# F-Fer/SLAM-Loop-Closing

Hardware: AMD Instinct MI355X
Metric: Hamming distances/sec (256-bit ORB) for all-vs-all loop search, 1/2/4/8 GPUs (higher is better)
Workload: dtype u32

## Files before the change

include/lcm.h:

```cpp
#ifndef LCM_H_
#define LCM_H_

#include <stddef.h>
#include <stdint.h>

#ifdef __cplusplus
extern "C" {
#endif

#if defined(__GNUC__)
#define LCM_API __attribute__((visibility("default")))
#else
#define LCM_API
#endif

#define LCM_DESC_BYTES 32
#define LCM_DESC_WORDS 8
#define LCM_MAX_TRAIN_ROWS (1 << 22)

typedef enum lcm_status {
    LCM_OK = 0,
    LCM_ERR_INVALID_ARG = -1,
    LCM_ERR_NO_DEVICE = -2,
    LCM_ERR_HIP = -3,
// ... 275 lines not shown
LCM_API int  lcm_group_sync(lcm_group* g);
LCM_API int  lcm_group_set_tuning(lcm_group* g, int knob, int value);
LCM_API int  lcm_group_set_kernel_variant(lcm_group* g, int variant);
LCM_API int  lcm_group_all_vs_all(lcm_group* g, lcm_score* out_scores, size_t cap, size_t* n_pairs, size_t* pair_offsets);
LCM_API int  lcm_group_all_vs_all_argmin(lcm_group* g, lcm_score* out_scores, uint32_t* out_index_sums, size_t cap,
                                         size_t* n_pairs, size_t* pair_offsets);
LCM_API int  lcm_group_all_vs_all_loops(lcm_group* g, lcm_loop_candidate* out, size_t cap, size_t* n_out, size_t* n_pairs_out);
LCM_API int  lcm_group_all_vs_all_ratio(lcm_group* g, double ratio, lcm_score* out_scores, size_t cap, size_t* n_pairs,
                                        size_t* pair_offsets);
LCM_API int  lcm_group_all_vs_all_loops_ratio(lcm_group* g, const lcm_ratio_loop_params* rp, lcm_loop_candidate* out,
                                              size_t cap, size_t* n_out, size_t* n_pairs_out);
LCM_API int  lcm_group_last_info(const lcm_group* g, lcm_group_info* info);
LCM_API int  lcm_group_query_scores(lcm_group* g, const uint8_t* query, int nq, int query_frame_id,
                                    lcm_score* out_scores, int32_t* out_frame_ids, int cap, int* n_out);
LCM_API int  lcm_group_query_scores_batch(lcm_group* g, const uint8_t* const* queries, const int* nq,
                                          const int* query_frame_ids, int n_queries,
                                          lcm_score* out_scores, size_t cap, size_t* n_out, size_t* offsets);
LCM_API int  lcm_group_query_submit_batch(lcm_group* g, const uint8_t* const* queries, const int* nq,
                                          const int* query_frame_ids, int n_queries, int* ticket);
LCM_API int  lcm_group_query_collect_batch(lcm_group* g, int ticket, lcm_score* out_scores, size_t cap, size_t* n_out,
                                           size_t* offsets);
LCM_API int  lcm_group_online_stats_read(lcm_group* g, lcm_online_stats* out, int reset);
LCM_API int  lcm_group_detect_loops(lcm_group* g, int current_frame_id, const uint8_t* query, int nq, int n_keypoints,
                                    lcm_loop_candidate* out, int cap, int* n_out);
LCM_API int  lcm_merge_shard_scores(const lcm_score* const* shard_scores, const size_t* shard_counts, int world,
                                    const int32_t* ids, int n_frames, int min_gap,
                                    lcm_score* out, size_t cap, size_t* n_out, size_t* offsets);

LCM_API int  lcm_merge_shard_scores_device(lcm_handle* h, const void* d_gathered, const size_t* shard_counts, int world,
                                           const int32_t* ids, int n_frames, int min_gap,
                                           void* d_merged, size_t cap, size_t* n_out);

typedef enum lcm_tuning { LCM_TUNE_ITEM_SLOTS = 0, LCM_TUNE_ONLINE_SPLIT = 1, LCM_TUNE_PACKED = 2, LCM_TUNE_ONLINE_STREAMS = 3,
                          LCM_TUNE_PACKED_SCRATCH_MB = 4, LCM_TUNE_PAIR_UPLOAD_KERNEL = 5, LCM_TUNE_PAIR_HOST_FOLD = 6 } lcm_tuning;
LCM_API int  lcm_set_tuning(lcm_handle* h, int knob, int value);

LCM_API int  lcm_dev_alloc(lcm_handle* h, size_t bytes, void** d_ptr);
LCM_API int  lcm_dev_free(lcm_handle* h, void* d_ptr);
LCM_API int  lcm_dev_upload(lcm_handle* h, void* d_dst, const void* src, size_t bytes);
LCM_API int  lcm_dev_download(lcm_handle* h, void* dst, const void* d_src, size_t bytes);

#ifdef __cplusplus
}
#endif
#endif
```

slam-loop-closing_amd/capi.py:

```python
from __future__ import annotations

import ctypes as C
import os
from typing import Optional, Sequence, Tuple

import numpy as np

_HERE = os.path.dirname(os.path.abspath(__file__))
LIB_PATH = os.environ.get("LCM_LIB_PATH") or os.path.join(_HERE, "lib", "liblcm_hip.so")
DESC_BYTES = 32
SIFT_BYTES = 128
KEY_SHIFT = 22
TUNE_ITEM_SLOTS, TUNE_ONLINE_SPLIT, TUNE_PACKED, TUNE_ONLINE_STREAMS, TUNE_PACKED_SCRATCH_MB = 0, 1, 2, 3, 4
TUNE_PAIR_UPLOAD_KERNEL, TUNE_PAIR_HOST_FOLD = 5, 6


OK, ERR_INVALID_ARG, ERR_NO_DEVICE, ERR_HIP, ERR_CAPACITY, ERR_ORDER, ERR_NOT_FOUND, ERR_OOM = 0, -1, -2, -3, -4, -5, -6, -7


class LcmError(RuntimeError):
    def __init__(self, code: int, msg: str):
        super().__init__(f"lcm error {code}: {msg}")
        self.code = code


class Params(C.Structure):
    _fields_ = [("ratio", C.c_int32), ("dist_floor", C.c_int32), ("min_matches", C.c_int32),
                ("min_gap", C.c_int32), ("sim_threshold", C.c_double), ("cross_check", C.c_int32),
                ("reserved", C.c_int32)]


class Score(C.Structure):
    _fields_ = [("good_count", C.c_uint32), ("min_dist", C.c_uint16), ("n_train", C.c_uint16)]


class DMatch(C.Structure):
    _fields_ = [("query_idx", C.c_int32), ("train_idx", C.c_int32), ("img_idx", C.c_int32), ("distance", C.c_float)]


class LoopCandidate(C.Structure):
    _fields_ = [("current_frame_id", C.c_int32), ("matched_frame_id", C.c_int32), ("num_matches", C.c_int32),
                ("similarity_score", C.c_double)]


class RatioLoopParams(C.Structure):
    _fields_ = [("ratio", C.c_double), ("min_rows", C.c_int32), ("min_matches", C.c_int32)]

# ... 1346 lines not shown
```

slam-loop-closing_amd/csrc/lcm_api.cpp:

```cpp
#include "lcm_internal.h"

namespace lcm {
std::string& last_error() { static thread_local std::string e; return e; }
int fail(int code, const char* fmt, ...) {
    char buf[512];
    va_list ap;
    va_start(ap, fmt);
    vsnprintf(buf, sizeof buf, fmt, ap);
    va_end(ap);
    last_error() = buf;
    return code;
}
void set_last_error(const char* msg) { last_error() = msg ? msg : ""; }
}

namespace lcm {

int set_device(const lcm_handle* h) {
    HIP_TRY(hipSetDevice(h->device));
    return LCM_OK;
}

int wait_db(lcm_handle* h) {
    if (h->pending_copy) {
// ... 247 lines not shown

int lcm_set_kernel_variant(lcm_handle* h, int variant) {
    if (!h) return fail(LCM_ERR_INVALID_ARG, "NULL handle");
    if (variant < 0 || variant > 5) return fail(LCM_ERR_INVALID_ARG, "unknown kernel variant %d", variant);
    h->variant = variant;
    return LCM_OK;
}

int lcm_set_tuning(lcm_handle* h, int knob, int value) {
    if (!h) return fail(LCM_ERR_INVALID_ARG, "NULL handle");
    switch (knob) {
        case LCM_TUNE_ITEM_SLOTS:
            if (value < 0 || value > 64) return fail(LCM_ERR_INVALID_ARG, "item slots must be 0 (automatic) .. 64");
            h->tune_item_slots = value; h->plan.key = 0; return LCM_OK;
        case LCM_TUNE_ONLINE_SPLIT:
            if (value != -1 && value != 0 && value != 1 && value != 2 && value != 4 && value != 16 && value != 32)
                return fail(LCM_ERR_INVALID_ARG, "online split must be -1 (automatic), 0 (off), 1, 2, 4 (rows per lane of a 256-thread workgroup), 16 or 32 (64 / 128 threads x 8 rows)");
            h->tune_online_split = value; return LCM_OK;
        case LCM_TUNE_ONLINE_STREAMS:
            if (value != 0 && value != 1) return fail(LCM_ERR_INVALID_ARG, "online streams must be 0 (the handle's stream) or 1 (one per query slot)");
            h->tune_online_streams = value; return LCM_OK;
        case LCM_TUNE_PAIR_UPLOAD_KERNEL:
            if (value != 0 && value != 1) return fail(LCM_ERR_INVALID_ARG, "pair upload must be 0 (hipMemcpyAsync) or 1 (kernel)");
            h->tune_pair_upload_kernel = value; return LCM_OK;
        case LCM_TUNE_PAIR_HOST_FOLD:
            if (value != 0 && value != 1) return fail(LCM_ERR_INVALID_ARG, "pair host fold must be 0 (device buffer + copy) or 1 (pinned host memory)");
            h->tune_pair_host_fold = value; return LCM_OK;
        case LCM_TUNE_PACKED_SCRATCH_MB:
            if (value < 1 || value > 65536) return fail(LCM_ERR_INVALID_ARG, "packed scratch must be 1 .. 65536 MiB per chunk");
            h->pk_scratch_cfg_words = h->pk_scratch_words = (size_t)value << 18; h->plan.key = 0; return LCM_OK;
        case LCM_TUNE_PACKED:
            if (value < -1 || value > 2) return fail(LCM_ERR_INVALID_ARG, "packed rows must be -1 (automatic), 0 (off), 1 (on) or 2 (on, 1536-row columns)");
            h->tune_packed = value; h->plan.key = 0; return LCM_OK;
        default: return fail(LCM_ERR_INVALID_ARG, "unknown tuning knob %d", knob);
    }
}


static int db_reserve_impl(lcm_handle* h, int n_frames, int max_desc) {
    if (!h || n_frames < 0 || max_desc < 0) return fail(LCM_ERR_INVALID_ARG, "bad argument");
    if (max_desc > MAX_FRAME_ROWS) return fail(LCM_ERR_CAPACITY, "a stored frame may hold at most %d rows (got %d)", MAX_FRAME_ROWS, max_desc);
    int rc = set_device(h); if (rc) return rc;
    return grow_arena(h, std::max(n_frames, 1), std::max(max_desc, 1));
}

static int db_append_impl(lcm_handle* h, int frame_id, const uint8_t* desc, int n, int n_keypoints) {
    if (!h || (n > 0 && !desc)) return fail(LCM_ERR_INVALID_ARG, "NULL argument");
    int rc = set_device(h); if (rc) return rc;
    rc = check_append(h, frame_id, n); if (rc) return rc;
    const int slot = (int)h->frames.size();
    const int b = h->stage_next;
    h->stage_next = (b + 1) % STAGE_BUFS;
    HIP_TRY(hipEventSynchronize(h->stage_done[b]));
    const int np = padded_rows(n);
    if (n > 0) {
        memcpy(h->h_stage[b], desc, (size_t)n * LCM_DESC_BYTES);
        for (int r = n; r < np; ++r) memcpy(h->h_stage[b] + (size_t)r * LCM_DESC_BYTES, desc + (size_t)(n - 1) * LCM_DESC_BYTES, LCM_DESC_BYTES);
        HIP_TRY(hipMemcpyAsync(h->d_rows + (size_t)slot * h->stride_rows * LCM_DESC_BYTES, h->h_stage[b],
                               (size_t)np * LCM_DESC_BYTES, hipMemcpyHostToDevice, h->copy_stream));
    }
    h->h_counts[slot] = n;
    HIP_TRY(hipMemcpyAsync(h->d_counts + slot, h->h_counts + slot, sizeof(int32_t), hipMemcpyHostToDevice, h->copy_stream));
    HIP_TRY(hipEventRecord(h->stage_done[b], h->copy_stream));
    HIP_TRY(hipEventRecord(h->db_ready, h->copy_stream));
    h->pending_copy = true; h->db_ready_recorded = true;
    h->frames.push_back({frame_id, n, n_keypoints < 0 ? n : n_keypoints});
// ... 259 lines not shown
```

slam-loop-closing_amd/csrc/lcm_bulk.cpp:

```cpp
#include "lcm_internal.h"

namespace {

struct PackedPlan {
    std::vector<uint32_t> tab;
    std::vector<lcm::WorkItem> items;
    std::vector<Plan::PackedChunk> chunks;
    size_t max_pairs = 0;
    uint64_t lane_slots = 0;
};

constexpr int PK_GROUP_FRAMES = 256;

int build_packed_plan(const std::vector<size_t>& offsets, const std::vector<int32_t>& qn, const uint32_t* q_frame_of, int chunk,
                      uint32_t COL, uint32_t stride, size_t scratch_words, PackedPlan& pk) {
    const size_t budget = std::max<size_t>(1, scratch_words / stride);
    const int n_q = (int)qn.size();
    auto elig_of = [&](int c) { return (uint32_t)(offsets[(size_t)c + 1] - offsets[(size_t)c]); };
    pk.tab.resize((size_t)n_q * 2 + 1);
    for (int c = 0; c <= n_q; ++c) pk.tab[(size_t)c] = (uint32_t)offsets[(size_t)c];
    for (int c = 0; c < n_q; ++c) pk.tab[(size_t)n_q + 1 + (size_t)c] = (uint32_t)qn[(size_t)c];
    std::vector<int> pos;
    struct Col { uint32_t w, k, me; };
    std::vector<Col> cols;
    bool first_chunk = offsets[(size_t)n_q] > budget;
    int c0 = 0;
    while (c0 < n_q) {
        const int min_frames = (int)std::max<size_t>(1, std::min<size_t>((size_t)PK_GROUP_FRAMES, budget / (size_t)std::max(chunk, 1)));
        int c1 = c0;
        size_t pairs = 0;
        while (c1 < n_q && (c1 - c0 < min_frames || pairs + elig_of(c1) <= budget)) { pairs += elig_of(c1); ++c1; }
        pos.clear();
        for (int c = c0; c < c1; ++c) if (elig_of(c) > 0) pos.push_back(c);
        c0 = c1;
        if (pos.empty()) continue;
        std::stable_sort(pos.begin(), pos.end(), [&](int x, int y) { return elig_of(x) > elig_of(y); });
        const size_t np = pos.size();
        const uint32_t tab0 = (uint32_t)pk.tab.size();
        pk.tab.resize(pk.tab.size() + 4 * np + 1);
        uint32_t* vstart = pk.tab.data() + tab0;
        uint32_t* qframe = vstart + np + 1;
        uint32_t* eligp = qframe + np;
        uint32_t* cidx = eligp + np;
        uint64_t v = 0;
// ... 26 lines not shown
            ch.item0 = (uint32_t)pk.items.size(); ch.tab0 = tab0; ch.ptab0 = (uint32_t)pk.tab.size(); ch.n_pos = (uint32_t)np; ch.slot0 = s0;
            pk.tab.resize(pk.tab.size() + np + 1);
            {
                uint32_t* pairsp = pk.tab.data() + ch.ptab0;
                size_t t = 0;
                for (size_t q = 0; q < np; ++q) {
                    pairsp[q] = (uint32_t)t;
                    const uint32_t e = pk.tab[tab0 + 2 * np + 1 + q];
                    if (e > s0) t += std::min(s1, e) - s0;
                }
                pairsp[np] = (uint32_t)t;
                ch.n_pairs = (uint32_t)t;
            }
            size_t live = cols.size();
            for (uint32_t bb = s0; bb < s1 && live > 0; bb += (uint32_t)chunk) {
                while (live > 0 && cols[live - 1].me <= bb) --live;
                for (size_t cc = 0; cc < live; ++cc)
                    pk.items.push_back({cols[cc].w, bb, std::min((uint32_t)chunk, std::min(s1, cols[cc].me) - bb), cols[cc].k});
            }
            ch.n_items = (uint32_t)pk.items.size() - ch.item0;
            if (ch.n_pairs > 0) {
                pk.chunks.push_back(ch);
                pk.max_pairs = std::max(pk.max_pairs, (size_t)ch.n_pairs);
                first_chunk = false;
            }
            s0 = s1;
        }
    }
    return LCM_OK;
}

int launch_packed(lcm_handle* h, const Plan& P, lcm::ScoreArgs a, bool argmin, void* d_scores, uint32_t* d_idx_sums) {
    const bool two = P.pk_chunks.size() > 1;
    const size_t half_words = P.pk_max_pairs * (size_t)P.pk_stride;
    const size_t need_words = half_words * (two ? 2 : 1);
    if (h->d_mdist && h->d_mdist_n > 4 * std::max<size_t>(need_words, (size_t)1 << 24)) {
        HIP_TRY(hipStreamSynchronize(h->stream));
        HIP_TRY(hipFree(h->d_mdist));
        h->d_mdist = nullptr; h->d_mdist_n = 0;
    }
    int rc = ensure_dev(h->d_mdist, h->d_mdist_n, need_words); if (rc) return rc;
    if (two && !h->stream2) {
        HIP_TRY(hipStreamCreateWithFlags(&h->stream2, hipStreamNonBlocking));
        HIP_TRY(hipEventCreateWithFlags(&h->ev_fork, hipEventDisableTiming));
        HIP_TRY(hipEventCreateWithFlags(&h->ev_join, hipEventDisableTiming));
    }
    HIP_TRY(hipEventRecord(h->ev_start, h->stream));
    if (two) {
        HIP_TRY(hipEventRecord(h->ev_fork, h->stream));
        HIP_TRY(hipStreamWaitEvent(h->stream2, h->ev_fork, 0));
    }
    h->fold_ev_used = 0;
    h->aux_pending = false;
    uint32_t launches = 0, biggest = 0;
    size_t k = 0;
    for (const Plan::PackedChunk& ch : P.pk_chunks) {
        hipStream_t st = (two && (k & 1)) ? h->stream2 : h->stream;
        uint32_t* scratch = h->d_mdist + ((two && (k & 1)) ? half_words : 0);
        ++k;
        a.items = P.d_items + ch.item0;
        a.pk_vstart = P.d_pk_tab + ch.tab0;
        a.pk_qframe = a.pk_vstart + ch.n_pos + 1;
        a.pk_elig = a.pk_qframe + ch.n_pos;
        a.pk_pairs = P.d_pk_tab + ch.ptab0; a.pk_slot0 = ch.slot0;
        a.pk_dist = scratch; a.pk_n = ch.n_pos; a.pk_col_rows = P.pk_col_rows; a.pk_stride = P.pk_stride;
        while (h->fold_ev.size() < h->fold_ev_used + 3) {
            hipEvent_t ev = nullptr;
            HIP_TRY(hipEventCreate(&ev));
            h->fold_ev.push_back(ev);
        }
        HIP_TRY(hipEventRecord(h->fold_ev[h->fold_ev_used], st));
        hipError_t e = lcm::launch_score_packed(a, ch.n_items, argmin, st);
        if (e != hipSuccess) return fail(LCM_ERR_HIP, "kernel launch failed: %s", hipGetErrorString(e));
        lcm::FinalizeBulkArgs f{};
        f.stride = P.pk_stride; f.key_shift = argmin ? lcm::KEY_SHIFT : 0; f.idx_sums = d_idx_sums;
        f.word_bytes = argmin ? 4 : 2;
        f.dist = scratch; f.offsets = P.d_pk_tab; f.nq = reinterpret_cast<const int32_t*>(P.d_pk_tab + P.pk_n_q + 1);
        f.db_counts = h->d_counts; f.scores = d_scores; f.n_q = P.pk_n_q; f.pair_base = 0;
        f.pk_pairs = a.pk_pairs; f.pk_cidx = a.pk_elig + ch.n_pos; f.pk_n = ch.n_pos; f.slot0 = ch.slot0;
        f.ratio = h->params.ratio; f.dist_floor = h->params.dist_floor;
        HIP_TRY(hipEventRecord(h->fold_ev[h->fold_ev_used + 1], st));
        e = lcm::launch_finalize_bulk(f, ch.n_pairs, st);
        if (e != hipSuccess) return fail(LCM_ERR_HIP, "fold kernel launch failed: %s", hipGetErrorString(e));
        HIP_TRY(hipEventRecord(h->fold_ev[h->fold_ev_used + 2], st));
        h->fold_ev_used += 3;
        launches += 2; biggest = std::max(biggest, ch.n_items);
    }
    if (two) {
        HIP_TRY(hipEventRecord(h->ev_join, h->stream2));
        HIP_TRY(hipStreamWaitEvent(h->stream, h->ev_join, 0));
    }
    HIP_TRY(hipEventRecord(h->ev_stop, h->stream));
    h->info_pending = true;
    h->info.launches = launches; h->info.workgroups = biggest; h->info.route = LCM_ROUTE_PACKED;
    h->info.launches_in_flight = two ? 2 : 1;
    h->info.pairs = P.n_pairs; h->info.distances = P.distances; h->info.algo_bytes = P.algo_bytes;
    return LCM_OK;
}

}

extern "C" {


static int all_vs_all_impl(lcm_handle* h, const void* d_query_rows, const int32_t* d_query_counts,
// ... 292 lines not shown
```

slam-loop-closing_amd/csrc/lcm_internal.h:

```cpp
#pragma once
#include "../../include/lcm.h"

#include <hip/hip_runtime.h>
#include <sys/stat.h>

#include <algorithm>
#include <cstdarg>
#include <cstdio>
#include <cstdlib>
#include <cstring>
#include <new>
#include <string>
#include <vector>

#include "lcm_kernels.h"

namespace lcm {
std::string& last_error();
int fail(int code, const char* fmt, ...) __attribute__((format(printf, 2, 3)));
void set_last_error(const char* msg);
}

namespace {
using lcm::fail;
// ... 94 lines not shown
    uint32_t pk_stride = 2048;
};

}

using lcm::FrameMeta;
using lcm::Plan;
using lcm::QuerySlot;

struct lcm_handle {
    lcm_params params;
    int device = 0;
    hipStream_t stream = nullptr;
    bool own_stream = false;
    hipStream_t copy_stream = nullptr;
    hipStream_t stream2 = nullptr;
    hipEvent_t ev_fork = nullptr, ev_join = nullptr;
    hipEvent_t db_ready = nullptr;
    hipEvent_t ev_start = nullptr, ev_stop = nullptr;
    hipEvent_t ev_aux_start = nullptr, ev_aux_stop = nullptr;
    bool aux_pending = false;
    std::vector<hipEvent_t> fold_ev;
    size_t fold_ev_used = 0;
    int variant = 0;
    int tune_item_slots = 0;
    int tune_online_split = -1;
    int tune_pair_upload_kernel = 1;
    int tune_pair_host_fold = 1;
    int tune_online_streams = 1;
    size_t pk_scratch_cfg_words = (size_t)1 << 28;
    size_t pk_scratch_words = (size_t)1 << 28;
    bool pk_oom_retry = false;
    int tune_packed = -1;

    uint8_t* d_rows = nullptr;
    int32_t* d_counts = nullptr;
    int cap_frames = 0;
    int stride_rows = 0;
    std::vector<FrameMeta> frames;
    bool pending_copy = false;
    bool db_ready_recorded = false;

    uint8_t* h_stage[lcm::STAGE_BUFS] = {nullptr, nullptr};
    size_t h_stage_bytes = 0;
    hipEvent_t stage_done[lcm::STAGE_BUFS] = {nullptr, nullptr};
    int32_t* h_counts = nullptr;
    int h_counts_cap = 0;
    int stage_next = 0;

    uint32_t* d_keys = nullptr; size_t d_keys_n = 0;
    uint8_t* h_pair_stage = nullptr; size_t h_pair_stage_bytes = 0;
    uint8_t* d_pair_stage = nullptr; size_t d_pair_stage_bytes = 0;
    uint32_t* h_final_keys = nullptr; size_t h_final_keys_n = 0;
    uint8_t* d_xq = nullptr; size_t d_xq_bytes = 0;
    uint8_t* d_pm1 = nullptr; size_t d_pm1_bytes = 0; uint64_t pm1_stamp = 0; size_t pm1_frames = 0;
    uint8_t* d_qpm1 = nullptr; size_t d_qpm1_bytes = 0;
    uint32_t* d_mdist = nullptr; size_t d_mdist_n = 0;
    uint8_t* d_mitems = nullptr; size_t d_mitems_bytes = 0;
    uint32_t* d_mmeta = nullptr; size_t d_mmeta_n = 0;
    lcm_score* d_bulk_scores = nullptr; size_t d_bulk_scores_n = 0;
    size_t bulk_scores_valid = 0;
    int32_t* d_meta = nullptr; size_t d_meta_n = 0;
    lcm_loop_candidate* d_cands = nullptr; size_t d_cands_n = 0;

    QuerySlot qslots[lcm::QUERY_SLOTS];
    lcm_online_stats online{};
// ... 161 lines not shown
```

slam-loop-closing_amd/csrc/lcm_kernels.h:

```cpp
#pragma once
#include <hip/hip_runtime.h>
#include <stdint.h>

namespace lcm {

constexpr int KEY_SHIFT = 22;
constexpr uint32_t KEY_IDX_MASK = (1u << KEY_SHIFT) - 1;
constexpr int MAX_FUSED_QUERY_ROWS = 2048;
constexpr int MAX_QUERY_BATCH = 16;

struct WorkItem {
    uint32_t q_frame;
    uint32_t slot_begin;
    uint32_t n_slots;
    uint32_t out_offset;
};

struct PairItem {
    uint32_t q_row;
    uint32_t t_row;
    uint32_t nq_nt;
    uint32_t out_offset;
};

// ... 2 lines not shown
    const int32_t*  q_counts;
    uint32_t        q_stride_words;
    const uint32_t* db_rows;
    const int32_t*  db_counts;
    uint32_t        db_stride_words;
    const WorkItem* items;
    const PairItem* pair_items;
    void*           scores;
    uint32_t*       keys;
    uint32_t        keys_stride;
    uint32_t*       idx_sums;
    int32_t         ratio;
    int32_t         dist_floor;
    uint32_t        imp_chunks, imp_chunk_rows, imp_spi, imp_total;
    int32_t         imp_nq;
    const uint32_t* pk_vstart;
    const uint32_t* pk_qframe;
    const uint32_t* pk_elig;
    const uint32_t* pk_pairs;
    uint32_t*       pk_dist;
    uint32_t        pk_n;
    uint32_t        pk_col_rows;
    uint32_t        pk_stride;
    uint32_t        pk_slot0;
    uint32_t        imp_nbatch;
    uint32_t        bat_wg[MAX_QUERY_BATCH + 1];
    uint32_t        bat_pair[MAX_QUERY_BATCH + 1];
    int32_t         bat_nq[MAX_QUERY_BATCH];
    uint32_t        bat_elig[MAX_QUERY_BATCH];
};

hipError_t launch_score(const ScoreArgs& a, uint32_t n_items, int max_query_rows, bool write_keys, int variant,
                        hipStream_t st);
hipError_t launch_score_packed(const ScoreArgs& a, uint32_t n_items, bool argmin, hipStream_t st);

hipError_t launch_score_split(const ScoreArgs& a, uint32_t n_items, int qpt, hipStream_t st);
struct FinalizeArgs {
    const uint32_t* dist;
    uint32_t        padded_rows;
    int32_t         nq;
    const int32_t*  db_counts;
    uint32_t        slot_begin;
    void*           scores;
    int32_t         ratio, dist_floor;
    uint32_t        n_batch;
    uint32_t        bat_pair[MAX_QUERY_BATCH + 1];
    int32_t         bat_nq[MAX_QUERY_BATCH];
};
hipError_t launch_finalize(const FinalizeArgs& a, uint32_t n_pairs, hipStream_t st);

struct PairDesc {
    uint32_t first_item;
    uint32_t n_seg;
    uint32_t seg_rows;
    uint32_t nq;
    uint32_t out_row0;
};
struct FoldArgs {
    const uint32_t* seg_keys;
    uint32_t        chunk_rows;
    const PairDesc* pairs;
    uint32_t*       final_keys;
    uint32_t        n_pairs;
    uint32_t        pair_base;
};
hipError_t grid_y_limit(uint32_t* limit);
hipError_t launch_fold_pair_keys(const FoldArgs& a, uint32_t max_nq, hipStream_t st);
// ... 233 lines not shown
```

slam-loop-closing_amd/csrc/lcm_kernels.hip:

```cpp
#include <hip/hip_runtime.h>
#include <stdint.h>

#include <algorithm>
#include <atomic>

#include "lcm_kernels.h"

#ifndef LCM_INNER_PRIO
#define LCM_INNER_PRIO 1
#endif

namespace lcm {

typedef const uint32_t __attribute__((address_space(4))) * sptr_t;
typedef const int32_t __attribute__((address_space(4))) * siptr_t;

__device__ __forceinline__ void fold2(uint32_t& best, const uint32_t (&q)[8], const uint32_t* s, uint32_t t0, uint32_t t1) {
#if LCM_INNER_PRIO
    uint32_t d0, d1, x0, x1;
    asm volatile(
        "v_xor_b32_e32 %3, %5, %21\n\tv_xor_b32_e32 %4, %13, %21\n\ts_setprio 3\n\t"
        "v_bcnt_u32_b32 %1, %3, 0\n\tv_bcnt_u32_b32 %2, %4, 0\n\ts_setprio 0\n\t"
        "v_xor_b32_e32 %3, %6, %22\n\tv_xor_b32_e32 %4, %14, %22\n\ts_setprio 3\n\t"
        "v_bcnt_u32_b32 %1, %3, %1\n\tv_bcnt_u32_b32 %2, %4, %2\n\ts_setprio 0\n\t"
// ... 69 lines not shown
        "v_bcnt_u32_b32 %1, %3, %1\n\tv_bcnt_u32_b32 %2, %4, %2\n\t"
        "v_min3_u32 %0, %0, %1, %2\n\ts_setprio 0"
        : "+v"(best), "=&v"(d0), "=&v"(d1), "=&v"(x0), "=&v"(x1)
        : "s"(s[0]), "s"(s[1]), "s"(s[2]), "s"(s[3]), "s"(s[4]), "s"(s[5]), "s"(s[6]), "s"(s[7]),
          "s"(s[8]), "s"(s[9]), "s"(s[10]), "s"(s[11]), "s"(s[12]), "s"(s[13]), "s"(s[14]), "s"(s[15]),
          "v"(q[0]), "v"(q[1]), "v"(q[2]), "v"(q[3]), "v"(q[4]), "v"(q[5]), "v"(q[6]), "v"(q[7]));
#else
    uint32_t d0, d1, x;
    asm volatile(
        "v_xor_b32_e32 %3, %4, %20\n\ts_nop 0\n\tv_bcnt_u32_b32 %1, %3, 0\n\t"
        "v_xor_b32_e32 %3, %5, %21\n\ts_nop 0\n\tv_bcnt_u32_b32 %1, %3, %1\n\t"
        "v_xor_b32_e32 %3, %6, %22\n\ts_nop 0\n\tv_bcnt_u32_b32 %1, %3, %1\n\t"
        "v_xor_b32_e32 %3, %7, %23\n\ts_nop 0\n\tv_bcnt_u32_b32 %1, %3, %1\n\t"
        "v_xor_b32_e32 %3, %8, %24\n\ts_nop 0\n\tv_bcnt_u32_b32 %1, %3, %1\n\t"
        "v_xor_b32_e32 %3, %9, %25\n\ts_nop 0\n\tv_bcnt_u32_b32 %1, %3, %1\n\t"
        "v_xor_b32_e32 %3, %10, %26\n\ts_nop 0\n\tv_bcnt_u32_b32 %1, %3, %1\n\t"
        "v_xor_b32_e32 %3, %11, %27\n\ts_nop 0\n\tv_bcnt_u32_b32 %1, %3, %1\n\t"
        "v_xor_b32_e32 %3, %12, %20\n\ts_nop 0\n\tv_bcnt_u32_b32 %2, %3, 0\n\t"
        "v_xor_b32_e32 %3, %13, %21\n\ts_nop 0\n\tv_bcnt_u32_b32 %2, %3, %2\n\t"
        "v_xor_b32_e32 %3, %14, %22\n\ts_nop 0\n\tv_bcnt_u32_b32 %2, %3, %2\n\t"
        "v_xor_b32_e32 %3, %15, %23\n\ts_nop 0\n\tv_bcnt_u32_b32 %2, %3, %2\n\t"
        "v_xor_b32_e32 %3, %16, %24\n\ts_nop 0\n\tv_bcnt_u32_b32 %2, %3, %2\n\t"
        "v_xor_b32_e32 %3, %17, %25\n\ts_nop 0\n\tv_bcnt_u32_b32 %2, %3, %2\n\t"
        "v_xor_b32_e32 %3, %18, %26\n\ts_nop 0\n\tv_bcnt_u32_b32 %2, %3, %2\n\t"
        "v_xor_b32_e32 %3, %19, %27\n\ts_nop 0\n\tv_bcnt_u32_b32 %2, %3, %2\n\t"
        "v_min3_u32 %0, %0, %1, %2"
        : "+v"(best), "=&v"(d0), "=&v"(d1), "=&v"(x)
        : "s"(s[0]), "s"(s[1]), "s"(s[2]), "s"(s[3]), "s"(s[4]), "s"(s[5]), "s"(s[6]), "s"(s[7]),
          "s"(s[8]), "s"(s[9]), "s"(s[10]), "s"(s[11]), "s"(s[12]), "s"(s[13]), "s"(s[14]), "s"(s[15]),
          "v"(q[0]), "v"(q[1]), "v"(q[2]), "v"(q[3]), "v"(q[4]), "v"(q[5]), "v"(q[6]), "v"(q[7]));
#endif
}

typedef uint32_t u32x4 __attribute__((ext_vector_type(4)));
__device__ __forceinline__ uint32_t rescan_distance(const uint32_t (&q)[8], const uint32_t* base, uint32_t off) {
    u32x4 lo, hi;
    asm volatile(
        "global_load_dwordx4 %0, %2, %3\n\t"
        "global_load_dwordx4 %1, %2, %3 offset:16\n\t"
        "s_waitcnt vmcnt(0)"
        : "=&v"(lo), "=&v"(hi)
        : "v"(off), "s"(base)
        : "memory");
    uint32_t d = __popc(q[0] ^ lo.x);
    d += __popc(q[1] ^ lo.y); d += __popc(q[2] ^ lo.z); d += __popc(q[3] ^ lo.w);
    d += __popc(q[4] ^ hi.x); d += __popc(q[5] ^ hi.y); d += __popc(q[6] ^ hi.z); d += __popc(q[7] ^ hi.w);
    return d;
}

constexpr int ARGMIN_GROUP = 8;

template <int THREADS, int QPT, int ARGMIN_MODE, bool WRITE_KEYS, bool PACKED = false>
__global__ __launch_bounds__(THREADS, (PACKED && QPT == 6) ? 8 : (ARGMIN_MODE == 2 ? 5 : 6)) void k_score_rowlane(ScoreArgs a) {
    constexpr bool ARGMIN = ARGMIN_MODE != 0;
    constexpr bool GROUPED = ARGMIN_MODE == 1;
    constexpr bool KEYED = ARGMIN_MODE == 2;
    constexpr int DSHIFT = ARGMIN ? KEY_SHIFT : 0;
    __shared__ uint32_t red_min[2];
    __shared__ uint32_t red_sum[2];
    __shared__ uint32_t red_idx[2];
    __shared__ uint32_t lane_key[(GROUPED || PACKED) ? THREADS * QPT : 1];
    __shared__ uint32_t lane_meta[PACKED ? THREADS * QPT : 1];

    const int tid = threadIdx.x;
    if (tid == 0) { red_min[0] = red_min[1] = 0xFFFFFFFFu; red_sum[0] = red_sum[1] = 0u; red_idx[0] = red_idx[1] = 0u; }
    __syncthreads();

    WorkItem it;
    int nq;
    size_t q_word0;
    uint32_t pair_t_row = 0;
    int pair_nt = -1;
    if (PACKED) {
        it = a.items[blockIdx.x];
        nq = (int)min((uint32_t)(THREADS * QPT), a.pk_vstart[a.pk_n] - it.q_frame * (uint32_t)(THREADS * QPT));
        q_word0 = 0;
    } else if (a.pair_items) {
        const PairItem pi = a.pair_items[blockIdx.x];
        it.q_frame = 0; it.slot_begin = 0; it.n_slots = 1; it.out_offset = pi.out_offset;
        nq = (int)(pi.nq_nt & 0xFFFu);
        pair_nt = (int)(pi.nq_nt >> 12);
        pair_t_row = pi.t_row;
        q_word0 = (size_t)pi.q_row * 8;
    } else if (a.items) {
        it = a.items[blockIdx.x];
        nq = a.q_counts[it.q_frame];
        q_word0 = (size_t)it.q_frame * a.q_stride_words;
    } else {
        uint32_t b = blockIdx.x, qi = 0, total = a.imp_total, pair0 = 0;
        int rows = a.imp_nq;
        if (a.imp_nbatch) {
            while (qi + 1 < a.imp_nbatch && b >= a.bat_wg[qi + 1]) ++qi;
            b -= a.bat_wg[qi];
            total = a.bat_elig[qi]; pair0 = a.bat_pair[qi]; rows = a.bat_nq[qi];
// ... 28 lines not shown
        for (int j = 0; j < QPT; ++j) {
            __builtin_amdgcn_sched_barrier(0);
            uint4 lo = make_uint4(0, 0, 0, 0), hi = make_uint4(0, 0, 0, 0);
            const uint32_t c = lane_meta[j * THREADS + tid];
            if (c != 0xFFFFFFFFu) {
                const uint32_t r = it.q_frame * (uint32_t)(THREADS * QPT) + (uint32_t)(j * THREADS + tid) - a.pk_vstart[c];
                const uint4* qb = reinterpret_cast<const uint4*>(a.q_rows + (size_t)a.pk_qframe[c] * a.q_stride_words);
                lo = qb[(size_t)r * 2]; hi = qb[(size_t)r * 2 + 1];
            }
            q[j][0] = lo.x; q[j][1] = lo.y; q[j][2] = lo.z; q[j][3] = lo.w;
            q[j][4] = hi.x; q[j][5] = hi.y; q[j][6] = hi.z; q[j][7] = hi.w;
        }
    } else {
        const uint4* qbase = reinterpret_cast<const uint4*>(a.q_rows + q_word0);
#pragma unroll
        for (int j = 0; j < QPT; ++j) {
            const int row = j * THREADS + tid;
            uint4 lo = make_uint4(0, 0, 0, 0), hi = make_uint4(0, 0, 0, 0);
            if (row < nq) { lo = qbase[row * 2]; hi = qbase[row * 2 + 1]; }
            q[j][0] = lo.x; q[j][1] = lo.y; q[j][2] = lo.z; q[j][3] = lo.w;
            q[j][4] = hi.x; q[j][5] = hi.y; q[j][6] = hi.z; q[j][7] = hi.w;
        }
    }

    for (uint32_t s = 0; s < it.n_slots; ++s) {
        const uint32_t slot = it.slot_begin + s;
        const int nt = pair_nt >= 0 ? pair_nt : ((siptr_t)a.db_counts)[slot];
        const uint32_t* Tbase = pair_nt >= 0 ? a.db_rows + (size_t)pair_t_row * 8 : a.db_rows + (size_t)slot * a.db_stride_words;
        sptr_t T = (sptr_t)Tbase;

        uint32_t best[QPT];
#pragma unroll
        for (int j = 0; j < QPT; ++j) best[j] = 0xFFFFFFFFu;
        if (GROUPED) {
#pragma unroll
            for (int j = 0; j < QPT; ++j) lane_key[j * THREADS + tid] = 0xFFFFFFFFu;
        }
        auto fold_group = [&](uint32_t g) {
#if LCM_INNER_PRIO
            __builtin_amdgcn_s_setprio(3);
#endif
#pragma unroll
            for (int j = 0; j < QPT; ++j) atomicMin(&lane_key[j * THREADS + tid], (best[j] << KEY_SHIFT) | g);
#if LCM_INNER_PRIO
            __builtin_amdgcn_s_setprio(0);
#endif
        };

        if (nt > 0) {
            uint32_t A[16], B[16];
#pragma unroll
            for (int k = 0; k < 16; ++k) A[k] = T[k];
            __builtin_amdgcn_s_waitcnt(0xC07F);
            for (int t = 0; t < nt; t += 4) {
#pragma unroll
                for (int k = 0; k < 16; ++k) B[k] = T[(t + 2) * 8 + k];
                __builtin_amdgcn_sched_barrier(0);
#pragma unroll
                for (int j = 0; j < QPT; ++j) {
                    if (KEYED) fold2(best[j], q[j], A, (uint32_t)t, (uint32_t)(t + 1)); else fold2_min(best[j], q[j], A);
                }
                __builtin_amdgcn_sched_barrier(0);
                __builtin_amdgcn_s_waitcnt(0xC07F);
#pragma unroll
                for (int k = 0; k < 16; ++k) A[k] = T[(t + 4) * 8 + k];
                __builtin_amdgcn_sched_barrier(0);
#pragma unroll
                for (int j = 0; j < QPT; ++j) {
                    if (KEYED) fold2(best[j], q[j], B, (uint32_t)(t + 2), (uint32_t)(t + 3)); else fold2_min(best[j], q[j], B);
                }
                __builtin_amdgcn_sched_barrier(0);
                if (GROUPED && (t & (ARGMIN_GROUP - 4)) == (ARGMIN_GROUP - 4)) fold_group((uint32_t)t / ARGMIN_GROUP);
                __builtin_amdgcn_s_waitcnt(0xC07F);
            }
            if (GROUPED) {
                fold_group((uint32_t)(nt - 1) / ARGMIN_GROUP);
                const uint32_t* Tg = Tbase;
                const uint32_t last_off = (uint32_t)(nt - 1) * 32u;
#pragma unroll
                for (int j = 0; j < QPT; ++j) {
                    __builtin_amdgcn_sched_barrier(0);
                    if (!valid(j)) continue;
                    const uint32_t row0 = (lane_key[j * THREADS + tid] & KEY_IDX_MASK) * ARGMIN_GROUP;
                    uint32_t kmin = 0xFFFFFFFFu;
#pragma unroll 1
                    for (uint32_t r = 0; r < (uint32_t)ARGMIN_GROUP; ++r) {
                        const uint32_t d = rescan_distance(q[j], Tg, min((row0 + r) * 32u, last_off));
                        kmin = min(kmin, (d << KEY_SHIFT) | (row0 + r));
                    }
                    lane_key[j * THREADS + tid] = kmin;
                }
                __builtin_amdgcn_sched_barrier(0);
            }
        }
        if (GROUPED && !PACKED) {
#pragma unroll
            for (int j = 0; j < QPT; ++j) best[j] = lane_key[j * THREADS + tid];
        }

        if (PACKED) {
            if (!GROUPED) {
#pragma unroll
                for (int j = 0; j < QPT; ++j) lane_key[j * THREADS + tid] = best[j];
            }
            __builtin_amdgcn_sched_barrier(0);
            uint32_t col0 = it.q_frame * (uint32_t)(THREADS * QPT);
            asm volatile("" : "+s"(col0));
#pragma unroll 1
            for (int j = 0; j < QPT; ++j) {
                const uint32_t c = lane_meta[j * THREADS + tid];
                if (c == 0xFFFFFFFFu) continue;
                const uint32_t r = col0 + (uint32_t)(j * THREADS + tid) - a.pk_vstart[c];
                if (slot < a.pk_elig[c]) {
                    const size_t w = ((size_t)a.pk_pairs[c] + (slot - a.pk_slot0)) * a.pk_stride + r;
                    if (GROUPED) a.pk_dist[w] = lane_key[j * THREADS + tid];
                    else reinterpret_cast<uint16_t*>(a.pk_dist)[w] = (uint16_t)lane_key[j * THREADS + tid];
                }
            }
            continue;
        }
        const size_t out = (size_t)it.out_offset + s;
        if (WRITE_KEYS) {
#pragma unroll
            for (int j = 0; j < QPT; ++j)
                if (valid(j)) a.keys[out * a.keys_stride + j * THREADS + tid] = best[j];
        }
        if (WRITE_KEYS && !ARGMIN) continue;
        const int par = s & 1;
        uint32_t dmin = 0xFFFFFFFFu;
#pragma unroll
        for (int j = 0; j < QPT; ++j) if (valid(j)) dmin = min(dmin, best[j] >> DSHIFT);
        atomicMin(&red_min[par], dmin);
        __syncthreads();
        dmin = red_min[par];
// ... 330 lines not shown
hipError_t launch_fold_pair_keys(const FoldArgs& a, uint32_t max_nq, hipStream_t st) {
    if (a.n_pairs == 0 || max_nq == 0) return hipSuccess;
    uint32_t lim = 0;
    hipError_t e = grid_y_limit(&lim);
    if (e != hipSuccess) return e;
    FoldArgs s = a;
    for (s.pair_base = 0; s.pair_base < a.n_pairs; s.pair_base += lim) {
        hipLaunchKernelGGL(k_fold_pair_keys, dim3((max_nq + 31) / 32, std::min(lim, a.n_pairs - s.pair_base)), dim3(256), 0, st, s);
        e = hipGetLastError();
        if (e != hipSuccess) return e;
        if (a.n_pairs - s.pair_base <= lim) break;
    }
    return hipSuccess;
}

__global__ __launch_bounds__(256) void k_upload_u4(uint4* __restrict__ dst, const uint4* __restrict__ src, uint32_t n16) {
    const uint32_t i = blockIdx.x * 256u + threadIdx.x;
    if (i < n16) dst[i] = src[i];
}

hipError_t launch_upload(void* d_dst, const void* h_src_pinned, size_t bytes, hipStream_t st) {
    const uint32_t n16 = (uint32_t)((bytes + 15) / 16);
    if (n16 == 0) return hipSuccess;
    hipLaunchKernelGGL(k_upload_u4, dim3((n16 + 255) / 256), dim3(256), 0, st, (uint4*)d_dst, (const uint4*)h_src_pinned, n16);
    return hipGetLastError();
}

hipError_t launch_finalize(const FinalizeArgs& a, uint32_t n_pairs, hipStream_t st) {
    if (n_pairs == 0) return hipSuccess;
    hipLaunchKernelGGL(k_finalize_pairs, dim3((n_pairs + 3) / 4), dim3(256), 0, st, a, n_pairs);
    return hipGetLastError();
}

hipError_t launch_score_packed(const ScoreArgs& a, uint32_t n_items, bool argmin, hipStream_t st) {
    if (n_items == 0) return hipSuccess;
    if (a.pk_col_rows == 1536) {
        if (argmin) hipLaunchKernelGGL((k_score_rowlane<256, 6, 1, false, true>), dim3(n_items), dim3(256), 0, st, a);
        else hipLaunchKernelGGL((k_score_rowlane<256, 6, 0, false, true>), dim3(n_items), dim3(256), 0, st, a);
        return hipGetLastError();
    }
    if (argmin) hipLaunchKernelGGL((k_score_rowlane<256, 8, 1, false, true>), dim3(n_items), dim3(256), 0, st, a);
    else hipLaunchKernelGGL((k_score_rowlane<256, 8, 0, false, true>), dim3(n_items), dim3(256), 0, st, a);
    return hipGetLastError();
}

hipError_t launch_score_pairs_small(const ScoreArgs& a, uint32_t n_items, hipStream_t st) {
    return launch_rowlane<256, 2>(a, n_items, true, true, st);
}

hipError_t launch_score_split(const ScoreArgs& a, uint32_t n_items, int qpt, hipStream_t st) {
    switch (qpt) {
        case 4: return launch_rowlane<256, 4>(a, n_items, true, false, st);
        case 2: return launch_rowlane<256, 2>(a, n_items, true, false, st);
        case 1: return launch_rowlane<256, 1>(a, n_items, true, false, st);
        case 16: return launch_rowlane<64, 8>(a, n_items, true, false, st);
        case 32: return launch_rowlane<128, 8>(a, n_items, true, false, st);
        default: return hipErrorInvalidValue;
    }
}

struct CandidateRec { int32_t cur, matched, num; int32_t pad; double sim; };
static_assert(sizeof(CandidateRec) == 24, "lcm_loop_candidate layout");

__device__ __forceinline__ bool loop_verdict(const LoopTestArgs& a, uint32_t p, CandidateRec& r) {
    if (p >= a.n_pairs) return false;
    uint32_t lo = 0, hi = a.n_q;
    while (hi - lo > 1) {
        const uint32_t mid = (lo + hi) >> 1;
        if (a.offsets[mid] <= p) lo = mid; else hi = mid;
    }
    const uint32_t c = lo, slot = p - a.offsets[c];
// ... 190 lines not shown
```

Baseline: 4316 billion.

## Keep packed-route running minima in LDS via ds_min instead of registers

Adds an LDS-minimum variant of the packed row-lane scoring kernel. The variant computes XOR/popcount distances in inline assembly and folds each result straight into per-lane LDS words with ds_min_u32, so the per-query running minima no longer occupy VGPRs. Group argmin keys are then built from those LDS words. The variant is selected by default when the packed column size equals the fused maximum, with a new tuning knob to switch it off. The aim is to free registers and shorten the VALU min chains, at the cost of extra LDS traffic, doubled LDS use for the argmin mode, and hand-placed waitcnts.

```diff
diff --git a/include/lcm.h b/include/lcm.h
--- a/include/lcm.h
+++ b/include/lcm.h
@@ -331,7 +331,8 @@
                                            void* d_merged, size_t cap, size_t* n_out);
 
 typedef enum lcm_tuning { LCM_TUNE_ITEM_SLOTS = 0, LCM_TUNE_ONLINE_SPLIT = 1, LCM_TUNE_PACKED = 2, LCM_TUNE_ONLINE_STREAMS = 3,
-                          LCM_TUNE_PACKED_SCRATCH_MB = 4, LCM_TUNE_PAIR_UPLOAD_KERNEL = 5, LCM_TUNE_PAIR_HOST_FOLD = 6 } lcm_tuning;
+                          LCM_TUNE_PACKED_SCRATCH_MB = 4, LCM_TUNE_PAIR_UPLOAD_KERNEL = 5, LCM_TUNE_PAIR_HOST_FOLD = 6,
+                          LCM_TUNE_PACKED_SCAN = 7 } lcm_tuning;
 LCM_API int  lcm_set_tuning(lcm_handle* h, int knob, int value);
 
 LCM_API int  lcm_dev_alloc(lcm_handle* h, size_t bytes, void** d_ptr);
diff --git a/slam-loop-closing_amd/capi.py b/slam-loop-closing_amd/capi.py
--- a/slam-loop-closing_amd/capi.py
+++ b/slam-loop-closing_amd/capi.py
@@ -12,7 +12,7 @@
 SIFT_BYTES = 128
 KEY_SHIFT = 22
 TUNE_ITEM_SLOTS, TUNE_ONLINE_SPLIT, TUNE_PACKED, TUNE_ONLINE_STREAMS, TUNE_PACKED_SCRATCH_MB = 0, 1, 2, 3, 4
-TUNE_PAIR_UPLOAD_KERNEL, TUNE_PAIR_HOST_FOLD = 5, 6
+TUNE_PAIR_UPLOAD_KERNEL, TUNE_PAIR_HOST_FOLD, TUNE_PACKED_SCAN = 5, 6, 7
 
 
 OK, ERR_INVALID_ARG, ERR_NO_DEVICE, ERR_HIP, ERR_CAPACITY, ERR_ORDER, ERR_NOT_FOUND, ERR_OOM = 0, -1, -2, -3, -4, -5, -6, -7
diff --git a/slam-loop-closing_amd/csrc/lcm_api.cpp b/slam-loop-closing_amd/csrc/lcm_api.cpp
--- a/slam-loop-closing_amd/csrc/lcm_api.cpp
+++ b/slam-loop-closing_amd/csrc/lcm_api.cpp
@@ -303,6 +303,9 @@
         case LCM_TUNE_PACKED:
             if (value < -1 || value > 2) return fail(LCM_ERR_INVALID_ARG, "packed rows must be -1 (automatic), 0 (off), 1 (on) or 2 (on, 1536-row columns)");
             h->tune_packed = value; h->plan.key = 0; return LCM_OK;
+        case LCM_TUNE_PACKED_SCAN:
+            if (value < -1 || value > 1) return fail(LCM_ERR_INVALID_ARG, "packed scan must be -1 (automatic), 0 (running minimum in registers) or 1 (in LDS words)");
+            h->tune_packed_scan = value; return LCM_OK;
         default: return fail(LCM_ERR_INVALID_ARG, "unknown tuning knob %d", knob);
     }
 }
diff --git a/slam-loop-closing_amd/csrc/lcm_bulk.cpp b/slam-loop-closing_amd/csrc/lcm_bulk.cpp
--- a/slam-loop-closing_amd/csrc/lcm_bulk.cpp
+++ b/slam-loop-closing_amd/csrc/lcm_bulk.cpp
@@ -10,6 +10,10 @@
     uint64_t lane_slots = 0;
 };
 
+#ifndef LCM_PACKED_SCAN_AUTO
+#define LCM_PACKED_SCAN_AUTO 1
+#endif
+constexpr int PACKED_SCAN_AUTO = LCM_PACKED_SCAN_AUTO;
 constexpr int PK_GROUP_FRAMES = 256;
 
 int build_packed_plan(const std::vector<size_t>& offsets, const std::vector<int32_t>& qn, const uint32_t* q_frame_of, int chunk,
@@ -102,6 +106,8 @@
 
 int launch_packed(lcm_handle* h, const Plan& P, lcm::ScoreArgs a, bool argmin, void* d_scores, uint32_t* d_idx_sums) {
     const bool two = P.pk_chunks.size() > 1;
+    const bool lds_min = P.pk_col_rows == (uint32_t)lcm::MAX_FUSED_QUERY_ROWS &&
+                         (h->tune_packed_scan < 0 ? PACKED_SCAN_AUTO : h->tune_packed_scan) == 1;
     const size_t half_words = P.pk_max_pairs * (size_t)P.pk_stride;
     const size_t need_words = half_words * (two ? 2 : 1);
     if (h->d_mdist && h->d_mdist_n > 4 * std::max<size_t>(need_words, (size_t)1 << 24)) {
@@ -140,7 +146,7 @@
             h->fold_ev.push_back(ev);
         }
         HIP_TRY(hipEventRecord(h->fold_ev[h->fold_ev_used], st));
-        hipError_t e = lcm::launch_score_packed(a, ch.n_items, argmin, st);
+        hipError_t e = lcm::launch_score_packed(a, ch.n_items, argmin, lds_min, st);
         if (e != hipSuccess) return fail(LCM_ERR_HIP, "kernel launch failed: %s", hipGetErrorString(e));
         lcm::FinalizeBulkArgs f{};
         f.stride = P.pk_stride; f.key_shift = argmin ? lcm::KEY_SHIFT : 0; f.idx_sums = d_idx_sums;
diff --git a/slam-loop-closing_amd/csrc/lcm_internal.h b/slam-loop-closing_amd/csrc/lcm_internal.h
--- a/slam-loop-closing_amd/csrc/lcm_internal.h
+++ b/slam-loop-closing_amd/csrc/lcm_internal.h
@@ -150,6 +150,7 @@
     size_t pk_scratch_words = (size_t)1 << 28;
     bool pk_oom_retry = false;
     int tune_packed = -1;
+    int tune_packed_scan = -1;
 
     uint8_t* d_rows = nullptr;
     int32_t* d_counts = nullptr;
diff --git a/slam-loop-closing_amd/csrc/lcm_kernels.h b/slam-loop-closing_amd/csrc/lcm_kernels.h
--- a/slam-loop-closing_amd/csrc/lcm_kernels.h
+++ b/slam-loop-closing_amd/csrc/lcm_kernels.h
@@ -58,7 +58,7 @@
 
 hipError_t launch_score(const ScoreArgs& a, uint32_t n_items, int max_query_rows, bool write_keys, int variant,
                         hipStream_t st);
-hipError_t launch_score_packed(const ScoreArgs& a, uint32_t n_items, bool argmin, hipStream_t st);
+hipError_t launch_score_packed(const ScoreArgs& a, uint32_t n_items, bool argmin, bool lds_min, hipStream_t st);
 
 hipError_t launch_score_split(const ScoreArgs& a, uint32_t n_items, int qpt, hipStream_t st);
 struct FinalizeArgs {
diff --git a/slam-loop-closing_amd/csrc/lcm_kernels.hip b/slam-loop-closing_amd/csrc/lcm_kernels.hip
--- a/slam-loop-closing_amd/csrc/lcm_kernels.hip
+++ b/slam-loop-closing_amd/csrc/lcm_kernels.hip
@@ -125,6 +125,36 @@
 #endif
 }
 
+template <int OFF>
+__device__ __forceinline__ void fold2_lds(uint32_t addr, const uint32_t (&q)[8], const uint32_t* s) {
+    uint32_t d0, d1, x0, x1;
+    asm volatile(
+        "v_xor_b32_e32 %2, %4, %20\n\tv_xor_b32_e32 %3, %12, %20\n\ts_setprio 3\n\t"
+        "v_bcnt_u32_b32 %0, %2, 0\n\tv_bcnt_u32_b32 %1, %3, 0\n\ts_setprio 0\n\t"
+        "v_xor_b32_e32 %2, %5, %21\n\tv_xor_b32_e32 %3, %13, %21\n\ts_setprio 3\n\t"
+        "v_bcnt_u32_b32 %0, %2, %0\n\tv_bcnt_u32_b32 %1, %3, %1\n\ts_setprio 0\n\t"
+        "v_xor_b32_e32 %2, %6, %22\n\tv_xor_b32_e32 %3, %14, %22\n\ts_setprio 3\n\t"
+        "v_bcnt_u32_b32 %0, %2, %0\n\tv_bcnt_u32_b32 %1, %3, %1\n\ts_setprio 0\n\t"
+        "v_xor_b32_e32 %2, %7, %23\n\tv_xor_b32_e32 %3, %15, %23\n\ts_setprio 3\n\t"
+        "v_bcnt_u32_b32 %0, %2, %0\n\tv_bcnt_u32_b32 %1, %3, %1\n\ts_setprio 0\n\t"
+        "v_xor_b32_e32 %2, %8, %24\n\tv_xor_b32_e32 %3, %16, %24\n\ts_setprio 3\n\t"
+        "v_bcnt_u32_b32 %0, %2, %0\n\tv_bcnt_u32_b32 %1, %3, %1\n\ts_setprio 0\n\t"
+        "v_xor_b32_e32 %2, %9, %25\n\tv_xor_b32_e32 %3, %17, %25\n\ts_setprio 3\n\t"
+        "v_bcnt_u32_b32 %0, %2, %0\n\tv_bcnt_u32_b32 %1, %3, %1\n\ts_setprio 0\n\t"
+        "v_xor_b32_e32 %2, %10, %26\n\tv_xor_b32_e32 %3, %18, %26\n\ts_setprio 3\n\t"
+        "v_bcnt_u32_b32 %0, %2, %0\n\tv_bcnt_u32_b32 %1, %3, %1\n\ts_setprio 0\n\t"
+        "v_xor_b32_e32 %2, %11, %27\n\tv_xor_b32_e32 %3, %19, %27\n\ts_setprio 3\n\t"
+        "v_bcnt_u32_b32 %0, %2, %0\n\tv_bcnt_u32_b32 %1, %3, %1\n\t"
+        "ds_min_u32 %28, %0 offset:%29\n\t"
+        "ds_min_u32 %28, %1 offset:%29\n\ts_setprio 0"
+        : "=&v"(d0), "=&v"(d1), "=&v"(x0), "=&v"(x1)
+        : "s"(s[0]), "s"(s[1]), "s"(s[2]), "s"(s[3]), "s"(s[4]), "s"(s[5]), "s"(s[6]), "s"(s[7]),
+          "s"(s[8]), "s"(s[9]), "s"(s[10]), "s"(s[11]), "s"(s[12]), "s"(s[13]), "s"(s[14]), "s"(s[15]),
+          "v"(q[0]), "v"(q[1]), "v"(q[2]), "v"(q[3]), "v"(q[4]), "v"(q[5]), "v"(q[6]), "v"(q[7]),
+          "v"(addr), "n"(OFF)
+        : "memory");
+}
+
 typedef uint32_t u32x4 __attribute__((ext_vector_type(4)));
 __device__ __forceinline__ uint32_t rescan_distance(const uint32_t (&q)[8], const uint32_t* base, uint32_t off) {
     u32x4 lo, hi;
@@ -145,14 +175,17 @@
 
 template <int THREADS, int QPT, int ARGMIN_MODE, bool WRITE_KEYS, bool PACKED = false>
 __global__ __launch_bounds__(THREADS, (PACKED && QPT == 6) ? 8 : (ARGMIN_MODE == 2 ? 5 : 6)) void k_score_rowlane(ScoreArgs a) {
-    constexpr bool ARGMIN = ARGMIN_MODE != 0;
-    constexpr bool GROUPED = ARGMIN_MODE == 1;
+    constexpr bool LDSMIN = ARGMIN_MODE == 3 || ARGMIN_MODE == 4;
+    static_assert(!LDSMIN || (PACKED && QPT == 8 && !WRITE_KEYS), "the LDS-minimum scan exists on the packed route only");
+    constexpr bool ARGMIN = ARGMIN_MODE != 0 && ARGMIN_MODE != 3;
+    constexpr bool GROUPED = ARGMIN_MODE == 1 || ARGMIN_MODE == 4;
     constexpr bool KEYED = ARGMIN_MODE == 2;
     constexpr int DSHIFT = ARGMIN ? KEY_SHIFT : 0;
     __shared__ uint32_t red_min[2];
     __shared__ uint32_t red_sum[2];
     __shared__ uint32_t red_idx[2];
-    __shared__ uint32_t lane_key[(GROUPED || PACKED) ? THREADS * QPT : 1];
+    constexpr int MINW = ARGMIN_MODE == 4 ? THREADS * QPT : 0;
+    __shared__ uint32_t lane_key[(GROUPED || PACKED) ? THREADS * QPT + MINW : 1];
     __shared__ uint32_t lane_meta[PACKED ? THREADS * QPT : 1];
 
     const int tid = threadIdx.x;
@@ -247,7 +280,12 @@
         uint32_t best[QPT];
 #pragma unroll
         for (int j = 0; j < QPT; ++j) best[j] = 0xFFFFFFFFu;
-        if (GROUPED) {
+        if constexpr (LDSMIN) {
+            uint32_t fresh = 0xFFFFFFFFu;
+            asm volatile("" : "+v"(fresh));
+#pragma unroll
+            for (int j = 0; j < (QPT * THREADS + MINW) / THREADS; ++j) lane_key[j * THREADS + tid] = fresh;
+        } else if (GROUPED) {
 #pragma unroll
             for (int j = 0; j < QPT; ++j) lane_key[j * THREADS + tid] = 0xFFFFFFFFu;
         }
@@ -255,8 +293,16 @@
 #if LCM_INNER_PRIO
             __builtin_amdgcn_s_setprio(3);
 #endif
-#pragma unroll
-            for (int j = 0; j < QPT; ++j) atomicMin(&lane_key[j * THREADS + tid], (best[j] << KEY_SHIFT) | g);
+            if constexpr (ARGMIN_MODE == 4) {
+                uint32_t m[QPT];
+#pragma unroll
+                for (int j = 0; j < QPT; ++j) m[j] = lane_key[MINW + j * THREADS + tid];
+#pragma unroll
+                for (int j = 0; j < QPT; ++j) atomicMin(&lane_key[j * THREADS + tid], (m[j] << KEY_SHIFT) | g);
+            } else {
+#pragma unroll
+                for (int j = 0; j < QPT; ++j) atomicMin(&lane_key[j * THREADS + tid], (best[j] << KEY_SHIFT) | g);
+            }
 #if LCM_INNER_PRIO
             __builtin_amdgcn_s_setprio(0);
 #endif
@@ -264,29 +310,86 @@
 
         if (nt > 0) {
             uint32_t A[16], B[16];
-#pragma unroll
-            for (int k = 0; k < 16; ++k) A[k] = T[k];
-            __builtin_amdgcn_s_waitcnt(0xC07F);
-            for (int t = 0; t < nt; t += 4) {
-#pragma unroll
-                for (int k = 0; k < 16; ++k) B[k] = T[(t + 2) * 8 + k];
-                __builtin_amdgcn_sched_barrier(0);
-#pragma unroll
-                for (int j = 0; j < QPT; ++j) {
-                    if (KEYED) fold2(best[j], q[j], A, (uint32_t)t, (uint32_t)(t + 1)); else fold2_min(best[j], q[j], A);
+            if constexpr (LDSMIN) {
+                const uint32_t addr = (uint32_t)(uintptr_t)(__attribute__((address_space(3))) uint32_t*)&lane_key[tid];
+                constexpr int W = THREADS * 4, M = MINW * 4;
+                constexpr bool CUT3 = GROUPED;
+#pragma unroll
+                for (int k = 0; k < 16; ++k) A[k] = T[k];
+                __builtin_amdgcn_s_waitcnt(0xC07F);
+                for (int t = 0; t < nt; t += 4) {
+                    const bool group_ends = GROUPED && (t & (ARGMIN_GROUP - 4)) == (ARGMIN_GROUP - 4);
+#pragma unroll
+                    for (int k = 0; k < 16; ++k) B[k] = T[(t + 2) * 8 + k];
+                    __builtin_amdgcn_sched_barrier(0);
+                    fold2_lds<M + 0 * W>(addr, q[0], A); fold2_lds<M + 1 * W>(addr, q[1], A); fold2_lds<M + 2 * W>(addr, q[2], A);
+                    __builtin_amdgcn_sched_barrier(0);
+                    if (CUT3) __builtin_amdgcn_s_waitcnt(0xC07F);
+                    __builtin_amdgcn_sched_barrier(0);
+                    fold2_lds<M + 3 * W>(addr, q[3], A);
+                    __builtin_amdgcn_sched_barrier(0);
+                    if (!CUT3) __builtin_amdgcn_s_waitcnt(0xC07F);
+                    __builtin_amdgcn_sched_barrier(0);
+                    fold2_lds<M + 4 * W>(addr, q[4], A); fold2_lds<M + 5 * W>(addr, q[5], A);
+                    fold2_lds<M + 6 * W>(addr, q[6], A); fold2_lds<M + 7 * W>(addr, q[7], A);
+                    __builtin_amdgcn_sched_barrier(0);
+                    __builtin_amdgcn_s_waitcnt(0xC07F);
+#pragma unroll
+                    for (int k = 0; k < 16; ++k) A[k] = T[(t + 4) * 8 + k];
+                    __builtin_amdgcn_sched_barrier(0);
+                    fold2_lds<M + 0 * W>(addr, q[0], B); fold2_lds<M + 1 * W>(addr, q[1], B);
+                    fold2_lds<M + 2 * W>(addr, q[2], B); fold2_lds<M + 3 * W>(addr, q[3], B);
+                    __builtin_amdgcn_sched_barrier(0);
+                    __builtin_amdgcn_s_waitcnt(0xC07F);
+                    __builtin_amdgcn_sched_barrier(0);
+                    fold2_lds<M + 4 * W>(addr, q[4], B); fold2_lds<M + 5 * W>(addr, q[5], B);
+                    fold2_lds<M + 6 * W>(addr, q[6], B); fold2_lds<M + 7 * W>(addr, q[7], B);
+                    __builtin_amdgcn_sched_barrier(0);
+                    uint32_t gmin[QPT];
+                    if constexpr (ARGMIN_MODE == 4) {
+                        __builtin_amdgcn_s_setprio(3);
+#pragma unroll
+                        for (int j = 0; j < QPT; ++j) gmin[j] = lane_key[MINW + j * THREADS + tid];
+                        __builtin_amdgcn_s_setprio(0);
+                    }
+                    __builtin_amdgcn_sched_barrier(0);
+                    __builtin_amdgcn_s_waitcnt(0xC07F);
+                    __builtin_amdgcn_sched_barrier(0);
+                    if constexpr (ARGMIN_MODE == 4) {
+                        if (group_ends) {
+                            __builtin_amdgcn_s_setprio(3);
+#pragma unroll
+                            for (int j = 0; j < QPT; ++j) atomicMin(&lane_key[j * THREADS + tid], (gmin[j] << KEY_SHIFT) | ((uint32_t)t / ARGMIN_GROUP));
+                            __builtin_amdgcn_s_setprio(0);
+                        }
+                    }
+                    __builtin_amdgcn_sched_barrier(0);
                 }
-                __builtin_amdgcn_sched_barrier(0);
+            } else {
+#pragma unroll
+                for (int k = 0; k < 16; ++k) A[k] = T[k];
                 __builtin_amdgcn_s_waitcnt(0xC07F);
-#pragma unroll
-                for (int k = 0; k < 16; ++k) A[k] = T[(t + 4) * 8 + k];
-                __builtin_amdgcn_sched_barrier(0);
-#pragma unroll
-                for (int j = 0; j < QPT; ++j) {
-                    if (KEYED) fold2(best[j], q[j], B, (uint32_t)(t + 2), (uint32_t)(t + 3)); else fold2_min(best[j], q[j], B);
+                for (int t = 0; t < nt; t += 4) {
+#pragma unroll
+                    for (int k = 0; k < 16; ++k) B[k] = T[(t + 2) * 8 + k];
+                    __builtin_amdgcn_sched_barrier(0);
+#pragma unroll
+                    for (int j = 0; j < QPT; ++j) {
+                        if (KEYED) fold2(best[j], q[j], A, (uint32_t)t, (uint32_t)(t + 1)); else fold2_min(best[j], q[j], A);
+                    }
+                    __builtin_amdgcn_sched_barrier(0);
+                    __builtin_amdgcn_s_waitcnt(0xC07F);
+#pragma unroll
+                    for (int k = 0; k < 16; ++k) A[k] = T[(t + 4) * 8 + k];
+                    __builtin_amdgcn_sched_barrier(0);
+#pragma unroll
+                    for (int j = 0; j < QPT; ++j) {
+                        if (KEYED) fold2(best[j], q[j], B, (uint32_t)(t + 2), (uint32_t)(t + 3)); else fold2_min(best[j], q[j], B);
+                    }
+                    __builtin_amdgcn_sched_barrier(0);
+                    if (GROUPED && (t & (ARGMIN_GROUP - 4)) == (ARGMIN_GROUP - 4)) fold_group((uint32_t)t / ARGMIN_GROUP);
+                    __builtin_amdgcn_s_waitcnt(0xC07F);
                 }
-                __builtin_amdgcn_sched_barrier(0);
-                if (GROUPED && (t & (ARGMIN_GROUP - 4)) == (ARGMIN_GROUP - 4)) fold_group((uint32_t)t / ARGMIN_GROUP);
-                __builtin_amdgcn_s_waitcnt(0xC07F);
             }
             if (GROUPED) {
                 fold_group((uint32_t)(nt - 1) / ARGMIN_GROUP);
@@ -314,7 +417,7 @@
         }
 
         if (PACKED) {
-            if (!GROUPED) {
+            if (!GROUPED && !LDSMIN) {
 #pragma unroll
                 for (int j = 0; j < QPT; ++j) lane_key[j * THREADS + tid] = best[j];
             }
@@ -711,11 +814,16 @@
     return hipGetLastError();
 }
 
-hipError_t launch_score_packed(const ScoreArgs& a, uint32_t n_items, bool argmin, hipStream_t st) {
+hipError_t launch_score_packed(const ScoreArgs& a, uint32_t n_items, bool argmin, bool lds_min, hipStream_t st) {
     if (n_items == 0) return hipSuccess;
     if (a.pk_col_rows == 1536) {
         if (argmin) hipLaunchKernelGGL((k_score_rowlane<256, 6, 1, false, true>), dim3(n_items), dim3(256), 0, st, a);
         else hipLaunchKernelGGL((k_score_rowlane<256, 6, 0, false, true>), dim3(n_items), dim3(256), 0, st, a);
+        return hipGetLastError();
+    }
+    if (lds_min) {
+        if (argmin) hipLaunchKernelGGL((k_score_rowlane<256, 8, 4, false, true>), dim3(n_items), dim3(256), 0, st, a);
+        else hipLaunchKernelGGL((k_score_rowlane<256, 8, 3, false, true>), dim3(n_items), dim3(256), 0, st, a);
         return hipGetLastError();
     }
     if (argmin) hipLaunchKernelGGL((k_score_rowlane<256, 8, 1, false, true>), dim3(n_items), dim3(256), 0, st, a);
```

After: 4252 billion. -1.5%, worse.
